# clevercool/ANT-Quantization

Measured on AMD Instinct MI355X. Metric: Gelements/s quant-dequant + achieved HBM GB/s %peak, 4-bit ANT, 1/8 MI355X, higher is better.
Workload: dtype f32; 1 GPU; headline: 32 x [4096,4096] bf16 weight tensors per GPU, ANT 4-bit signed flint grid, calibrated per-row alpha, steady-state _forward; one step = ONE batched launch (antq_fakequant_batch) over all 32 tensors; io_dtype=bf16

## Files before the change

### ant_quantization_amd/_lib.py

```python
import ctypes
import os
import threading

import numpy as np
import torch

_HERE = os.path.dirname(os.path.abspath(__file__))
LIB_PATH = os.environ.get("ANTQ_LIB") or os.path.join(_HERE, "libantq.so")

ABI_VERSION = 7
F32, BF16, F16, F64 = 0, 1, 2, 3
FLAG_OVP = 1
FLAG_DYNAMIC = 2
FLAG_UNORDERED = 4
IDX_NONE = -1
IDX_VICTIM = -2
MAX_GRID = 1024
PLAN_MAX_BYTES = 128 + 4 * MAX_GRID + 16 * 3072 + 20 * 1024 + 16 * 64

_DTYPES = {torch.float32: F32, torch.bfloat16: BF16, torch.float16: F16, torch.float64: F64}

_lib = None
_lock = threading.RLock()

# ... 799 lines not shown
            else:
                batched.append(j)
        self.n_batched = len(batched)
        self.host = self.dev = None
        if batched:
            arr = (_Job * len(batched))()
            for k, (x, out, alpha, plan, gmax, rows, row_len, per_row) in enumerate(batched):
                arr[k] = _Job(x.data_ptr(), out.data_ptr(), alpha.data_ptr() if alpha is not None else 0, rows, row_len,
                              1 if per_row else 0, gmax,
                              plan.host_addr, plan.dev(self.device).data_ptr())
            cap = lib().antq_batch_capacity(arr, len(batched), self.dtype)
            host = np.zeros(cap, dtype=np.uint8)
            n = lib().antq_batch_build(arr, len(batched), self.dtype,
                                       (FLAG_OVP if ovp else 0) | (FLAG_DYNAMIC if dynamic else 0),
                                       host.ctypes.data_as(ctypes.c_void_p), ctypes.c_size_t(cap))
            if n <= 0:
                _check(n, "antq_batch_build")
            self.host = host[:n].copy()
            self.dev = torch.from_numpy(self.host).to(self.device)

    def run(self):
        e = _ext_mod if _ext_mod is not False else ext()
        if self.host is not None and e is not None:
            e.batch_run(self.host.ctypes.data, self.dev)
        elif self.host is not None:
            with _on_device(self.device):
                rc = lib().antq_fakequant_batch(ctypes.c_void_p(self.host.ctypes.data), ctypes.c_void_p(self.dev.data_ptr()),
                                                ctypes.c_void_p(_stream_int(self.device)))
            if rc:
                _check(rc, "antq_fakequant_batch")
        for x, out, alpha, plan, gmax, rows, row_len, per_row in self.singles:
            fakequant(x, alpha, plan, gmax, rows, row_len, per_row, ovp=self.ovp, out=out)

    def kernels(self):
        out = []
        if self.host is not None:
            h = self.host[:80].view(np.uint32)
            fam, pad = [int(v) for v in h[8:17]], int(h[17])
            t = {F32: "float", BF16: "bf16", F16: "f16"}[self.dtype]
            o = "true" if self.ovp else "false"
            dyn = "true" if int(h[3]) & FLAG_DYNAMIC else "false"
            if pad & 1:
                out.append(("antq::k_fq_batch_all<%s,%s>" % (t, o), fam[0]))
            elif fam[0]:
                w = 1 if ((pad >> 8) & 7) == 1 else 4
                out.append(("antq::k_fq_batch<%s,%s,%d>" % (t, o, w), fam[0] * (4 // w)))
            if fam[5]:
                out.append(("antq::k_fq_hbatch<%s,%s>" % (t, o), fam[5] * 4))
            for f, v in ((6, 1), (7, 4), (8, 16)):
                if fam[f] and not (pad & 1):
                    out.append(("antq::k_fq_hbatch_dyn<%s,%s,%d>" % (t, o, v), fam[f]))
            if not (pad & 1):
                if fam[1]:
                    out.append(("antq::k_fq_batch_d<%s,%s,true,%s>" % (t, o, dyn), fam[1]))
                if fam[2]:
                    out.append(("antq::k_fq_batch_d<%s,%s,false,%s>" % (t, o, dyn), fam[2]))
                if fam[3]:
                    out.append(("antq::k_fq_batch_dyn<%s,%s>" % (t, o), fam[3]))
                if fam[4]:
                    out.append(("antq::k_fq_batch_dyn16<%s,%s>" % (t, o), fam[4]))
        out += [("antq_fakequant (own launch)", 0)] * len(self.singles)
        return out
```

### ant_quantization_amd/csrc/antq_batch.hip

```cpp
#include "antq_host.h"
#include "antq_k_batch.h"

using namespace antq;

extern "C" size_t antq_batch_capacity(const antq_job *jobs, int n, int dtype)
{
    const int epl = epl_of(dtype);
    if (!jobs || n < 1 || !epl) return 0;
    size_t blocks = 0;
    for (int i = 0; i < n; i++) blocks += std::max(4 * job_blocks(jobs[i], epl, nullptr) + 1, jobs[i].rows);
    return sizeof(BatchHeader) + sizeof(BatchDesc) * (size_t)n + 4 * blocks;
}

extern "C" int antq_batch_build(const antq_job *jobs, int n, int dtype, unsigned flags, void *blob, size_t cap)
{
    const int epl = epl_of(dtype);
    if (!jobs || !blob || n < 1 || n > 65535) return ANTQ_ERR_ARG;
    if (!epl) return ANTQ_ERR_UNSUPPORTED;
    const bool dyn = (flags & ANTQ_FLAG_DYNAMIC) != 0;
    char *p = static_cast<char *>(blob);
    BatchHeader h;
    memset(&h, 0, sizeof(h));
    h.magic = kBatchMagic; h.n = (uint32_t)n; h.dtype = (uint32_t)dtype; h.flags = flags;
    h.map_offset = (uint32_t)(sizeof(BatchHeader) + sizeof(BatchDesc) * (size_t)n);
// ... 19 lines not shown
        if (!plan_args_from_host(J.plan_host, d.pa)) return ANTQ_ERR_PLAN;
        const PlanHeader *ph = static_cast<const PlanHeader *>(J.plan_host);
        const bool xdom = g_knob_x && d.pa.kind == kPlanLut && ph->xdom;
        d.vout = ph->vout;
        {
            const XArgs xe = xargs_from_plan(J.plan_host, d.pa);
            d.vmin = xe.vmin; d.vmax = xe.vmax;
        }
        d.ratio = 1.0f;
        int f;
        d.u = (uint32_t)kBatchU;
        if (!dyn) {
            if (d.kind == 0 && d.pa.adom && (dtype == ANTQ_F32 || g_knob_lane_rows == 2) && g_knob_lane_rows != 0) {
                d.kind = 1; d.total_tasks = 0; d.tpr = 1; d.vshift = -1;
                if ((d.vpr & (d.vpr - 1u)) == 0u) { d.vshift = 0; while ((1u << d.vshift) < d.vpr) d.vshift++; }
                blocks = (size_t)((d.n_vec + 256u * kBatchU - 1u) / (256u * kBatchU));
            }
            HArgs hx;
            const uint32_t hu = (d.kind == 0 && g_knob_h != 0 && hargs_from_plan(J.plan_host, dtype, J.gmax, hx))
                                    ? (g_knob_h == 2 ? row_task_u(d.vpr) : hrow_static_u(d.vpr, xdom)) : 0u;
            if (hu != 0u) {
                d.kind = 13;
                d.u = hu;
                if (g_knob_u >= 2 && g_knob_u <= 4) d.u = (uint32_t)g_knob_u;
                d.tpr = (d.vpr + 64u * d.u - 1u) / (64u * d.u);
                const size_t total = (J.alpha_per_row ? J.rows : (size_t)1) * (size_t)d.tpr;
                if (total > 0xfffffff0ull) return ANTQ_ERR_UNSUPPORTED;
                d.total_tasks = (uint32_t)total;
                blocks = (total + 3) / 4;
                d.rot = (d.vpr % (64u * d.u) != 0u && (d.tpr % 2u) == 0u) ? 1u : 0u;
                d.tlist = plan_tlist_dev(J.plan_host, J.plan_dev);
                d.h_n = hx.n_thr | (hx.n_neg << 16);
                d.hshift = hx.hshift;
            }
            if (d.kind == 0 && xdom) {
                d.kind = 2;
                d.u = row_task_u_small(d.vpr);
                if (g_knob_u >= 1 && g_knob_u <= 4) d.u = (uint32_t)g_knob_u;
                d.tpr = (d.vpr + 64u * d.u - 1u) / (64u * d.u);
                const size_t total = (J.alpha_per_row ? J.rows : (size_t)1) * (size_t)d.tpr;
                if (total > 0xfffffff0ull) return ANTQ_ERR_UNSUPPORTED;
                d.total_tasks = (uint32_t)total;
                blocks = (total + 3) / 4;
                d.rot = (d.vpr % (64u * d.u) != 0u && (d.tpr % 2u) == 0u) ? 1u : 0u;
            }
            f = d.kind == 13 ? 5 : d.kind == 2 ? 0 : (d.kind == 3 ? -1 : (d.pa.adom ? 1 : 2));
        } else {
            if (!J.alpha_per_row || d.kind == 3 || J.rows > 0x3ffffff0ull) return ANTQ_ERR_UNSUPPORTED;
            HArgs hprobe;
            const bool h_dyn = d.kind == 0 && g_knob_h != 0 && d.vpr <= 8192u && hargs_from_plan(J.plan_host, dtype, J.gmax, hprobe);
            if (!h_dyn && d.kind == 0 && d.pa.adom && dtype != ANTQ_F32 && d.vpr == 128u && g_knob_u != 1) {
                d.kind = 1; d.total_tasks = 0; d.tpr = 1; d.vshift = 7;
                blocks = (size_t)((d.n_vec + 256u * kBatchU - 1u) / (256u * kBatchU));
            }
            const HArgs &hx = hprobe;
            if (h_dyn) {
                const HDynShape sh = hrow_dyn_shape(d.vpr);
                d.kind = sh.wpr == 1 ? 14 : (sh.wpr == 4 ? 15 : 16);
                d.u = (uint32_t)sh.vpt;
                d.tpr = (uint32_t)sh.wpr;
                d.total_tasks = (uint32_t)(J.rows * (size_t)sh.wpr);
                blocks = sh.wpr == 1 ? (J.rows + 3) / 4 : J.rows;
                d.tlist = plan_tlist_dev(J.plan_host, J.plan_dev);
                d.h_n = hx.n_thr | (hx.n_neg << 16);
                d.hshift = hx.hshift;
                f = sh.wpr == 1 ? 6 : (sh.wpr == 4 ? 7 : 8);
// ... 30 lines not shown
        d.inv_gmax = 1.0 / (double)J.gmax;
        descs[i] = d;
        fam[(size_t)i] = (uint8_t)(f < 0 ? 255 : f);
        nblk[(size_t)i] = blocks;
        if (f == 1 || f == 2 || f < 0) lds = std::max(lds, lds_table(d.pa, false));
    }
    for (int i = 0; i < n; i++)
        if (fam[(size_t)i] == 255) fam[(size_t)i] = any_da ? 1 : 2;
    {
        size_t all_blocks = 0;
        for (int i = 0; i < n; i++) all_blocks += nblk[(size_t)i];
        const bool small = g_knob_u == 2 || (g_knob_u != 4 && (all_blocks < 4u * 2048u || dtype == ANTQ_F32));
        for (int i = 0; i < n && small; i++) {
            BatchDesc &d = descs[i];
            if (d.kind == 1 && d.pa.adom && !(dyn && d.vpr > 64u)) {
                d.u = 2u;
                nblk[(size_t)i] = (size_t)((d.n_vec + 511u) / 512u);
            }
        }
    }
    if (!dyn) {
        double h_bytes = 0.0;
        for (int i = 0; i < n; i++)
            if (fam[(size_t)i] == 5) h_bytes += 2.0 * (double)jobs[i].rows * (double)jobs[i].row_len * (dtype == ANTQ_F32 ? 4.0 : 2.0);
        const bool h_apart = h_bytes >= 128.0 * 1048576.0;
        if (!h_apart) {
            for (int i = 0; i < n; i++) {
                BatchDesc &d = descs[i];
                if (d.kind != 13) continue;
                bool other = false;
                for (int k = 0; k < n && !other; k++) other = fam[(size_t)k] != 5;
                if (!other) break;
                const PlanHeader *ph = static_cast<const PlanHeader *>(jobs[i].plan_host);
                if (g_knob_x && d.pa.kind == kPlanLut && ph->xdom) {
                    d.kind = 2;
                    d.u = row_task_u_small(d.vpr);
                    d.tpr = (d.vpr + 64u * d.u - 1u) / (64u * d.u);
                    d.total_tasks = (uint32_t)((jobs[i].alpha_per_row ? jobs[i].rows : (size_t)1) * (size_t)d.tpr);
                    d.rot = (d.vpr % (64u * d.u) != 0u && (d.tpr % 2u) == 0u) ? 1u : 0u;
                    fam[(size_t)i] = 0;
                } else {
                    const size_t tpr = (d.vpr + 64 * kBatchU - 1) / (64 * kBatchU);
                    d.kind = 0; d.u = (uint32_t)kBatchU; d.tpr = (uint32_t)tpr; d.rot = 0;
                    d.total_tasks = (uint32_t)((jobs[i].alpha_per_row ? jobs[i].rows : (size_t)1) * tpr);
                    lds = std::max(lds, lds_table(d.pa, false));
                    fam[(size_t)i] = (uint8_t)(d.pa.adom ? 1 : 2);
                }
                nblk[(size_t)i] = ((size_t)d.total_tasks + 3) / 4;
            }
        }
        bool seen[kBatchFamilies] = {false, false, false, false, false, false, false, false, false};
        int nf_rest = 0;
        for (int i = 0; i < n; i++)
            if (fam[(size_t)i] != 5 && !seen[fam[(size_t)i]]) { seen[fam[(size_t)i]] = true; nf_rest++; }
        if (nf_rest > 1) {
            h.pad = 1u;
            for (int i = 0; i < n; i++)
                if (fam[(size_t)i] != 5) fam[(size_t)i] = 0;
        }
    }
    {
        double long_b = 0.0, short_b = 0.0;
        for (int i = 0; i < n; i++)
            if (descs[i].kind == 2) (descs[i].vpr >= 256u ? long_b : short_b) += (double)descs[i].total_tasks * descs[i].u;
        h.pad |= ((long_b >= short_b && !big_footprint) ? 1u : 4u) << 8;
    }
    {
        uint32_t umax = 0;
        for (int i = 0; i < n; i++)
            if (descs[i].kind == 14) umax = std::max(umax, descs[i].u);
        h.pad2[0] = hrow_dyn_lds_pad(HDynShape{1, (int)umax});
    }
    size_t total_blocks = 0;
    for (int i = 0; i < n; i++) {
        descs[i].first_block = (uint32_t)fam_blocks[fam[(size_t)i]];
        fam_blocks[fam[(size_t)i]] += nblk[(size_t)i];
        total_blocks += nblk[(size_t)i];
    }
    if (total_blocks > 0x1fffffffull) return ANTQ_ERR_UNSUPPORTED;
    if (cap < h.map_offset + 4 * total_blocks) return ANTQ_ERR_PLAN;
    size_t off[kBatchFamilies], acc = 0;
    for (int f = 0; f < kBatchFamilies; f++) { off[f] = acc; acc += fam_blocks[f]; h.fam_blocks[f] = (uint32_t)fam_blocks[f]; }
    for (int i = 0; i < n; i++) {
        uint32_t *m = map + off[fam[(size_t)i]] + descs[i].first_block;
        for (size_t b = 0; b < nblk[(size_t)i]; b++) m[b] = (uint32_t)i;
    }
    h.total_blocks = (uint32_t)total_blocks;
    h.lds_bytes = (uint32_t)lds;
    h.bytes = (uint32_t)(h.map_offset + 4 * total_blocks);
    memcpy(p, &h, sizeof(h));
    return (int)h.bytes;
}

template <typename T>
static void launch_hbatch(uint32_t map_entries, const BatchDesc *descs, const uint32_t *map, bool ovp, hipStream_t st)
{
    const dim3 g(map_entries * 4u), b(64u);
    const unsigned pad = g_knob_hlds >= 0 ? (unsigned)g_knob_hlds : (map_entries >= 8192u ? kHRowLdsPad : 0u);
    if (ovp) hipLaunchKernelGGL((k_fq_hbatch<T, true>), g, b, pad, st, descs, map, (uint32_t)g_knob_rot);
    else hipLaunchKernelGGL((k_fq_hbatch<T, false>), g, b, pad, st, descs, map, (uint32_t)g_knob_rot);
}
template <>
void launch_hbatch<float>(uint32_t, const BatchDesc *, const uint32_t *, bool, hipStream_t) {}

template <typename T>
static void launch_hbatch_dyn(const BatchHeader *h, const BatchDesc *descs, const uint32_t *const *fmap, bool ovp, hipStream_t st)
{
    if (h->fam_blocks[6]) {
        const dim3 g(h->fam_blocks[6] * 4u), b(64u);
        const unsigned pad = g_knob_hlds >= 0 ? (unsigned)g_knob_hlds : h->pad2[0];
        if (ovp) hipLaunchKernelGGL((k_fq_hbatch_dyn<T, true, 1>), g, b, pad, st, descs, fmap[6]);
        else hipLaunchKernelGGL((k_fq_hbatch_dyn<T, false, 1>), g, b, pad, st, descs, fmap[6]);
    }
    if (h->fam_blocks[7]) {
        const dim3 g(h->fam_blocks[7]), b(256u);
        if (ovp) hipLaunchKernelGGL((k_fq_hbatch_dyn<T, true, 4>), g, b, 0, st, descs, fmap[7]);
        else hipLaunchKernelGGL((k_fq_hbatch_dyn<T, false, 4>), g, b, 0, st, descs, fmap[7]);
    }
    if (h->fam_blocks[8]) {
        const dim3 g(h->fam_blocks[8]), b(1024u);
        if (ovp) hipLaunchKernelGGL((k_fq_hbatch_dyn<T, true, 16>), g, b, 0, st, descs, fmap[8]);
        else hipLaunchKernelGGL((k_fq_hbatch_dyn<T, false, 16>), g, b, 0, st, descs, fmap[8]);
    }
}
template <>
void launch_hbatch_dyn<float>(const BatchHeader *, const BatchDesc *, const uint32_t *const *, bool, hipStream_t) {}

extern "C" int antq_fakequant_batch(const void *batch_host, const void *batch_dev, void *stream)
{
    if (!batch_host || !batch_dev) return ANTQ_ERR_ARG;
    const BatchHeader *h = static_cast<const BatchHeader *>(batch_host);
    if (h->magic != kBatchMagic) return ANTQ_ERR_PLAN;
    if (h->total_blocks == 0) return ANTQ_OK;
    const char *pd = static_cast<const char *>(batch_dev);
    const BatchDesc *descs = reinterpret_cast<const BatchDesc *>(pd + sizeof(BatchHeader));
    const uint32_t *map = reinterpret_cast<const uint32_t *>(pd + h->map_offset);
    hipStream_t st = static_cast<hipStream_t>(stream);
    const dim3 block(256);
    const bool ovp = (h->flags & ANTQ_FLAG_OVP) != 0;
    const bool dyn = (h->flags & ANTQ_FLAG_DYNAMIC) != 0;
    const uint32_t *fmap[kBatchFamilies];
    {
        const uint32_t *m = map;
        for (int f = 0; f < kBatchFamilies; f++) { fmap[f] = m; m += h->fam_blocks[f]; }
    }
#define ANTQ_LAUNCH_D(TT, OO, AA)                                                                                   \
    do {                                                                                                            \
        const int f_ = (AA) ? 1 : 2;                                                                                \
         \
        const unsigned cap_ = (sizeof(TT) == 4 && !dyn && h->fam_blocks[f_] >= 32768u && h->lds_bytes < 24576u) ? 24576u - h->lds_bytes : 0u;  \
        const unsigned lds_ = h->lds_bytes + (g_knob_dlds >= 0 ? (unsigned)g_knob_dlds : cap_);                    \
        if (dyn) hipLaunchKernelGGL((k_fq_batch_d<TT, OO, AA, true>), dim3(h->fam_blocks[f_]), block, lds_, st, descs, fmap[f_]);  \
        else hipLaunchKernelGGL((k_fq_batch_d<TT, OO, AA, false>), dim3(h->fam_blocks[f_]), block, lds_, st, descs, fmap[f_]);     \
    } while (0)
#define ANTQ_LAUNCH_B(TT)                                                                                         \
    do {                                                                                                          \
        if (h->pad & 1u) {                                             \
            if (ovp) hipLaunchKernelGGL((k_fq_batch_all<TT, true>), dim3(h->fam_blocks[0]), block, h->lds_bytes, st, descs, fmap[0]);  \
            else hipLaunchKernelGGL((k_fq_batch_all<TT, false>), dim3(h->fam_blocks[0]), block, h->lds_bytes, st, descs, fmap[0]);     \
            if (h->fam_blocks[5]) launch_hbatch<TT>(h->fam_blocks[5], descs, fmap[5], ovp, st);    \
            break;                                                                                                \
        }                                                                                                         \
        if (h->fam_blocks[0]) {                                                                                   \
            const int hw_ = (int)((h->pad >> 8) & 7u);                                                           \
            const int w_ = (g_knob_waves == 4 || g_knob_waves == 2 || g_knob_waves == 1) ? g_knob_waves : (hw_ == 1 ? 1 : 4);   \
            const dim3 g_(h->fam_blocks[0] * (4u / w_)), b_(64u * w_);                                           \
            const uint32_t rot_ = (uint32_t)g_knob_rot;                                                          \
            if (w_ == 1) { if (ovp) hipLaunchKernelGGL((k_fq_batch<TT, true, 1>), g_, b_, 0, st, descs, fmap[0], rot_);        \
                           else hipLaunchKernelGGL((k_fq_batch<TT, false, 1>), g_, b_, 0, st, descs, fmap[0], rot_); }         \
            else if (w_ == 2) { if (ovp) hipLaunchKernelGGL((k_fq_batch<TT, true, 2>), g_, b_, 0, st, descs, fmap[0], rot_);   \
                           else hipLaunchKernelGGL((k_fq_batch<TT, false, 2>), g_, b_, 0, st, descs, fmap[0], rot_); }         \
            else { if (ovp) hipLaunchKernelGGL((k_fq_batch<TT, true, 4>), g_, b_, 0, st, descs, fmap[0], rot_);                \
                   else hipLaunchKernelGGL((k_fq_batch<TT, false, 4>), g_, b_, 0, st, descs, fmap[0], rot_); }                 \
        }                                                                                                         \
        if (h->fam_blocks[5]) launch_hbatch<TT>(h->fam_blocks[5], descs, fmap[5], ovp, st);                       \
        if (h->fam_blocks[6] || h->fam_blocks[7] || h->fam_blocks[8]) launch_hbatch_dyn<TT>(h, descs, fmap, ovp, st);      \
        if (h->fam_blocks[1]) { if (ovp) ANTQ_LAUNCH_D(TT, true, true); else ANTQ_LAUNCH_D(TT, false, true); }    \
        if (h->fam_blocks[2]) { if (ovp) ANTQ_LAUNCH_D(TT, true, false); else ANTQ_LAUNCH_D(TT, false, false); }  \
        if (h->fam_blocks[3]) {                                                                                   \
            if (ovp) hipLaunchKernelGGL((k_fq_batch_dyn<TT, true>), dim3(h->fam_blocks[3]), block, 0, st, descs, fmap[3]);   \
            else hipLaunchKernelGGL((k_fq_batch_dyn<TT, false>), dim3(h->fam_blocks[3]), block, 0, st, descs, fmap[3]);      \
        }                                                                                                         \
        if (h->fam_blocks[4]) {                                                                                   \
            if (ovp) hipLaunchKernelGGL((k_fq_batch_dyn16<TT, true>), dim3(h->fam_blocks[4]), dim3(1024), 0, st, descs, fmap[4]);   \
            else hipLaunchKernelGGL((k_fq_batch_dyn16<TT, false>), dim3(h->fam_blocks[4]), dim3(1024), 0, st, descs, fmap[4]);      \
        }                                                                                                         \
    } while (0)
    switch (h->dtype) {
    case ANTQ_F32: ANTQ_LAUNCH_B(float); break;
    case ANTQ_BF16: ANTQ_LAUNCH_B(bf16_tag); break;
    case ANTQ_F16: ANTQ_LAUNCH_B(f16_tag); break;
    default: return ANTQ_ERR_UNSUPPORTED;
    }
#undef ANTQ_LAUNCH_B
#undef ANTQ_LAUNCH_D
    return hipGetLastError() == hipSuccess ? ANTQ_OK : ANTQ_ERR_LAUNCH;
}

namespace antq {
int prefetch_unit_batch()
{
    hipFuncAttributes at;
    return hipFuncGetAttributes(&at, reinterpret_cast<const void *>(&k_fq_hbatch<bf16_tag, false>)) == hipSuccess ? ANTQ_OK : ANTQ_ERR_LAUNCH;
}
}
```

### ant_quantization_amd/csrc/antq_k_batch.h

```cpp
#ifndef ANTQ_K_BATCH_H
#define ANTQ_K_BATCH_H

#include "antq_k_fakequant.h"
#include "antq_k_hrow.h"

namespace antq {

constexpr uint32_t kBatchMagic = 0x33544E41u;
constexpr int kBatchU = 4;

struct BatchDesc {
    const uint4 *x;
    uint4 *out;
    const float *alpha;
    const uint4 *plan_tab;
    uint64_t n_vec;
    uint32_t total_tasks;
    uint32_t vpr;
    uint32_t tpr;
    int32_t vshift;
    uint32_t first_block;
    uint32_t kind;
    int32_t per_row;
    float gmax;
    PlanArgs pa;
    float vout;
    float ratio;
    uint32_t u;
    uint32_t rot;
    float vmin, vmax;
    uint32_t pad_;
    double inv_gmax;
    const uint4 *tlist;
    uint32_t h_n;
    uint32_t hshift;
};
static_assert(sizeof(BatchDesc) == 192, "BatchDesc must be 192 bytes");

constexpr int kBatchFamilies = 9;

struct BatchHeader {
    uint32_t magic, n, dtype, flags, lds_bytes, map_offset, bytes, total_blocks;
    uint32_t fam_blocks[kBatchFamilies];
    uint32_t pad;
    uint32_t pad2[2];
};
static_assert(sizeof(BatchHeader) == 80, "BatchHeader must be 80 bytes");

__device__ __forceinline__ XArgs xargs_of(const BatchDesc &D)
{
    const PlanArgs &pa = D.pa;
    XArgs xa;
    xa.m = pa.m; xa.shift = pa.shift; xa.kmin = pa.kmin; xa.kmax = pa.kmax; xa.keymask = pa.keymask;
    xa.nbneg = pa.nbneg; xa.n_entries = pa.n_entries; xa.xlim = pa.xlim; xa.vout = D.vout;
    xa.linear = pa.linear; xa.lin_scale = pa.lin_scale; xa.lin_bias = pa.lin_bias;
    xa.flim = pa.fastlim * 0.99999f; xa.vmin = D.vmin; xa.vmax = D.vmax; xa.inv_gmax = D.inv_gmax;
    return xa;
}

#ifndef ANTQ_OVP_WAVES
#define ANTQ_OVP_WAVES 8
#endif
#ifndef ANTQ_PLAIN_WAVES
#define ANTQ_PLAIN_WAVES 6
#endif
template <typename T, bool OVP, int WAVES = 4>
__global__ void __launch_bounds__(64 * WAVES, OVP ? ANTQ_OVP_WAVES : ANTQ_PLAIN_WAVES)
k_fq_batch(const BatchDesc *__restrict__ descs, const uint32_t *__restrict__ block_map, uint32_t rotate)
{
    constexpr uint32_t SPLIT = 4u / WAVES;
    uint32_t blk = blockIdx.x;
    if (WAVES < 4) {
        const uint32_t g8 = blk >> 3;
        if ((g8 << 3) + 8u <= gridDim.x && (rotate == 1u || (rotate == 0u && descs[block_map[(g8 << 3) / SPLIT]].rot)))
            blk = (g8 << 3) + ((blk + g8) & 7u);
    }
    const uint32_t b4 = blk / SPLIT, sub = blk % SPLIT;
    const uint32_t j = block_map[b4];
    const BatchDesc &D = descs[j];
    const uint32_t lb = b4 - D.first_block;
    const uint32_t lane = threadIdx.x & 63u;
    const uint32_t wv = threadIdx.x >> 6;
    const uint4 *plan_tab = D.plan_tab;
    const XArgs xa = xargs_of(D);

    __shared__ __attribute__((aligned(16))) uint4 wtab_all[WAVES][256];
    const uint32_t task = __builtin_amdgcn_readfirstlane(lb * 4u + sub * WAVES + wv);
    if (task >= D.total_tasks) return;
#define ANTQ_XROW(UU)                                                                                                   \
    xrow_task<T, OVP, false, UU, false, 1>(D.x, D.out, nullptr, task, D.vpr, D.tpr, D.alpha, D.per_row, D.gmax, 1.0f, nullptr, \
                                           xa, plan_tab + (D.pa.m_pad >> 2), reinterpret_cast<const float *>(plan_tab),        \
                                           wtab_all[wv], lane, wv)
    if (D.u == 4u) ANTQ_XROW(4); else if (D.u == 3u) ANTQ_XROW(3); else if (D.u == 1u) ANTQ_XROW(1); else ANTQ_XROW(2);
#undef ANTQ_XROW
}

template <typename T, bool OVP>
__global__ void __launch_bounds__(64)
k_fq_hbatch(const BatchDesc *__restrict__ descs, const uint32_t *__restrict__ block_map, uint32_t rotate)
{
    __shared__ __attribute__((aligned(16))) uint2 tab[kHSlots * 2];
    uint32_t blk = blockIdx.x;
    const uint32_t g8 = blk >> 3;
    if ((g8 << 3) + 8u <= gridDim.x && (rotate == 1u || (rotate == 0u && descs[block_map[(g8 << 3) >> 2]].rot)))
        blk = (g8 << 3) + ((blk + g8) & 7u);
    const uint32_t b4 = blk >> 2, sub = blk & 3u;
    const BatchDesc &D = descs[block_map[b4]];
    const uint32_t task = (b4 - D.first_block) * 4u + sub;
    if (task >= D.total_tasks) return;
    HArgs ha;
    ha.n_thr = D.h_n & 0xffffu; ha.n_neg = D.h_n >> 16; ha.hshift = D.hshift; ha.m = D.pa.m;
    ha.flim = D.pa.fastlim * 0.99999f; ha.lim = fminf(ha.flim, D.pa.xlim);
    ha.vmin = D.vmin; ha.vmax = D.vmax; ha.vout = D.vout; ha.inv_gmax = D.inv_gmax;
    const float *grid = reinterpret_cast<const float *>(D.plan_tab);
#define ANTQ_HROW(UU) hrow_wave_task<T, OVP, UU>(D.x, D.out, task, D.vpr, D.tpr, D.alpha, D.per_row, D.gmax, ha, D.tlist, grid, tab, threadIdx.x)
    if (D.u == 4u) ANTQ_HROW(4); else if (D.u == 3u) ANTQ_HROW(3); else ANTQ_HROW(2);
#undef ANTQ_HROW
}

template <typename T, bool OVP, int WPR>
__global__ void __launch_bounds__(64 * WPR)
k_fq_hbatch_dyn(const BatchDesc *__restrict__ descs, const uint32_t *__restrict__ block_map)
{
    __shared__ __attribute__((aligned(16))) uint2 tab[WPR][kHSlots * 2];
    const uint32_t wv = threadIdx.x >> 6, lane = threadIdx.x & 63u;
    const uint32_t ent = WPR == 1 ? (blockIdx.x >> 2) : blockIdx.x;
    const BatchDesc &D = descs[block_map[ent]];
    const uint32_t rowi = WPR == 1 ? (ent - D.first_block) * 4u + (blockIdx.x & 3u) : ent - D.first_block;
    if (rowi * (uint32_t)WPR >= D.total_tasks) return;
    const uint32_t task = __builtin_amdgcn_readfirstlane(rowi * WPR + wv);
    HArgs ha;
    ha.n_thr = D.h_n & 0xffffu; ha.n_neg = D.h_n >> 16; ha.hshift = D.hshift; ha.m = D.pa.m;
    ha.flim = D.pa.fastlim * 0.99999f; ha.lim = fminf(ha.flim, D.pa.xlim);
    ha.vmin = D.vmin; ha.vmax = D.vmax; ha.vout = D.vout; ha.inv_gmax = D.inv_gmax;
    const float *grid = reinterpret_cast<const float *>(D.plan_tab);
    float *alpha_out = const_cast<float *>(D.alpha);
    hrow_wave_task_dyn<T, OVP, WPR>(D.x, D.out, task, D.vpr, D.u, D.ratio, alpha_out, D.gmax, ha, D.tlist, grid, tab[wv], lane, wv);
}

template <typename T, bool OVP, bool AD, bool DYN>
__global__ void __launch_bounds__(256)
k_fq_batch_d(const BatchDesc *__restrict__ descs, const uint32_t *__restrict__ block_map)
{
    constexpr int U = kBatchU;
    extern __shared__ __attribute__((aligned(16))) uint4 smem[];
    const uint32_t j = block_map[blockIdx.x];
    const BatchDesc &D = descs[j];
    const PlanArgs pa = D.pa;
    const uint32_t lb = blockIdx.x - D.first_block;
// ... 207 lines not shown
```

### ant_quantization_amd/csrc/antq_k_hrow.h

```cpp
#ifndef ANTQ_K_HROW_H
#define ANTQ_K_HROW_H

#include "antq_k_fakequant.h"

namespace antq {

constexpr uint32_t kHNoThr = 0xffffffffu;
constexpr uint32_t kHSentinel = 0xffffu;

struct HArgs {
    uint32_t n_thr;
    uint32_t n_neg;
    uint32_t hshift;
    uint32_t m;
    float lim;
    float flim;
    float vmin, vmax;
    float vout;
    double inv_gmax;
};

template <typename T> struct H16;
template <> struct H16<bf16_tag> {
    static constexpr uint32_t MANT = 7;
// ... 78 lines not shown
    }
    __builtin_amdgcn_fence(__ATOMIC_RELEASE, "wavefront");
    __builtin_amdgcn_wave_barrier();
    __builtin_amdgcn_s_waitcnt(0xc07f);
    return R;
}

__device__ __forceinline__ uint32_t hrow_pair(uint32_t w, uint32_t tbase, uint32_t vkmin, uint32_t vklim, uint32_t kpos,
                                               uint32_t vkwid)
{
    uint32_t th, tl, wl, o;
    uint2 eh, el;
    asm("v_bfe_u32 %0, %1, %2, %3" : "=v"(th) : "v"(w), "s"(kpos), "v"(vkwid));
    asm("v_med3_i32 %0, %1, %2, %3" : "=v"(th) : "v"(th), "v"(vkmin), "v"(vklim));
    wl = w << 16;
    th = __builtin_amdgcn_alignbit(th, w, 31);
    asm("v_bfe_u32 %0, %1, %2, %3" : "=v"(tl) : "v"(wl), "s"(kpos), "v"(vkwid));
    asm("v_med3_i32 %0, %1, %2, %3" : "=v"(tl) : "v"(tl), "v"(vkmin), "v"(vklim));
    tl = __builtin_amdgcn_alignbit(tl, wl, 31);
    typedef unsigned int u32x2_t __attribute__((ext_vector_type(2)));
    const u32x2_t rh = *(const __attribute__((address_space(3))) u32x2_t *)(uintptr_t)((th << 3) + tbase);
    const u32x2_t rl = *(const __attribute__((address_space(3))) u32x2_t *)(uintptr_t)((tl << 3) + tbase);
    eh = make_uint2(rh.x, rh.y);
    el = make_uint2(rl.x, rl.y);
    asm("v_cmp_ge_u32 vcc, %1, %2\n\t"
        "v_cndmask_b32_sdwa %0, %3, %3, vcc dst_sel:DWORD dst_unused:UNUSED_PAD src0_sel:WORD_0 src1_sel:WORD_1"
        : "=&v"(o) : "v"(wl), "v"(el.x), "v"(el.y) : "vcc");
    asm("v_cmp_ge_u32 vcc, %1, %2\n\t"
        "v_cndmask_b32_sdwa %0, %3, %3, vcc dst_sel:WORD_1 dst_unused:UNUSED_PRESERVE src0_sel:WORD_0 src1_sel:WORD_1"
        : "+v"(o) : "v"(w), "v"(eh.x), "v"(eh.y) : "vcc");
    return o;
}

__device__ __forceinline__ uint32_t vec_word(const uint4 &v, int i) { return i == 0 ? v.x : (i == 1 ? v.y : (i == 2 ? v.z : v.w)); }
__device__ __forceinline__ void vec_set(uint4 &v, int i, uint32_t w)
{
    if (i == 0) v.x = w; else if (i == 1) v.y = w; else if (i == 2) v.z = w; else v.w = w;
}

template <typename T, bool OVP>
__device__ __forceinline__ uint4 hrow_exact(const uint4 &v, float s, const float *__restrict__ grid, uint32_t m)
{
    uint4 o = v;
#pragma unroll 1
    for (int i = 0; i < 4; i++) {
        const uint32_t w = vec_word(v, i);
        const float x0 = H16<T>::val(w & 0xffffu), x1 = H16<T>::val(w >> 16);
        const float d0 = x0 / s, d1 = x1 / s;
        float q0 = 0.0f, q1 = 0.0f, m0 = 102400.0f, m1 = 102400.0f;
#pragma unroll 1
        for (uint32_t k = 0; k < m; k++) {
            const float g = ld_global(grid + k);
            const float s0 = fabsf(d0 - g), s1 = fabsf(d1 - g);
            if (s0 <= m0) { m0 = s0; q0 = g; }
            if (s1 <= m1) { m1 = s1; q1 = g; }
        }
        if (OVP) {
            const bool me = fabsf(q0) > 32.0f, mo = fabsf(q1) > 32.0f;
            q0 = q0 * ((mo && !me) ? 0.0f : 1.0f);
            q1 = q1 * (me ? 0.0f : 1.0f);
        }
        const float t0 = (q0 - d0) + d0, t1 = (q1 - d1) + d1;
        vec_set(o, i, H16<T>::out(t0 * s) | (H16<T>::out(t1 * s) << 16));
    }
    return o;
}

__device__ __forceinline__ uint32_t hrow_victims(uint32_t o, uint32_t othr)
{
    const uint32_t mg = o & 0x7fff7fffu;
    const bool me = (mg & 0xffffu) >= othr, mo = (mg >> 16) >= othr;
    return o & (((mo && !me) ? 0u : 0xffffu) | (me ? 0u : 0xffff0000u));
}

struct HFar { float rs, flim, vmin, vmax; };

template <typename T, bool OVP>
__device__ __forceinline__ uint4 hrow_vec_far(const uint4 &v, uint32_t tbase, uint32_t vkmin, uint32_t vklim, uint32_t kpos,
                                              uint32_t vkwid, uint32_t othr, float s, const HFar &far,
                                              const float *__restrict__ grid, uint32_t m)
{
    uint4 o = v;
    bool decided = true;
#pragma unroll 1
    for (int i = 0; i < 4; i++) {
        const uint32_t w = vec_word(v, i);
        uint32_t ow = hrow_pair(w, tbase, vkmin, vklim, kpos, vkwid);
#pragma unroll
        for (int hf = 0; hf < 2; hf++) {
            if (((ow >> (16 * hf)) & 0xffffu) == kHSentinel) {
                const float xe = H16<T>::val((w >> (16 * hf)) & 0xffffu);
                decided = decided && (fabsf(xe * far.rs) < far.flim);
                const float d = xe / s;
                const float q = (d > 0.0f ? far.vmax : far.vmin) + 0.0f;
                const float t = (q - d) + d;
                const uint32_t pat = H16<T>::out(t * s);
                ow = hf ? ((ow & 0xffffu) | (pat << 16)) : ((ow & 0xffff0000u) | pat);
            }
        }
        if (OVP) ow = hrow_victims(ow, othr);
        vec_set(o, i, ow);
    }
    if (!decided) return hrow_exact<T, OVP>(v, s, grid, m);
    return o;
}

template <typename T, bool OVP, int VPT>
__device__ __forceinline__ void hrow_task(const uint4 (&v)[VPT], uint4 *__restrict__ out, uint32_t v0, uint32_t vpr,
                                          const HRow &R, uint32_t tab_addr, uint32_t hshift, uint32_t othr, float s,
                                          const HFar &far, const float *__restrict__ grid, uint32_t m, uint32_t nv = VPT)
{
    const uint32_t kpos = 16u + hshift;
    uint32_t vkmin = R.kmin, vklim = R.klim, vkwid = 15u - hshift;
    asm volatile("" : "+v"(vkmin), "+v"(vklim), "+v"(vkwid));
    const uint32_t tbase = tab_addr - (R.kmin << 4);
    if (R.fast) {
        u16x2_t acc = as_u16x2(0u);
#pragma unroll
        for (int u = 0; u < VPT; u++) {
            if ((uint32_t)u < nv && v0 + 64u * u < vpr) {
                const uint32_t w[4] = {v[u].x, v[u].y, v[u].z, v[u].w};
                uint32_t o[4];
#pragma unroll
                for (int i = 0; i < 4; i++) {
                    o[i] = hrow_pair(w[i], tbase, vkmin, vklim, kpos, vkwid);
                    acc = __builtin_elementwise_max(acc, as_u16x2(o[i]));
                    if (OVP) o[i] = hrow_victims(o[i], othr);
                }
                st_stream(out + 64u * u, make_uint4(o[0], o[1], o[2], o[3]));
            }
            __builtin_amdgcn_sched_barrier(0);
        }
        const uint32_t na = ~as_u32(acc);
        if (__builtin_expect((na & 0xffffu) != 0u && (na >> 16) != 0u, 1)) return;
    }
    const uint32_t slot0 = R.klim << hshift;
#pragma unroll 1
    for (uint32_t u = 0; u < nv; u++) {
        uint4 cur = v[0];
#pragma unroll
        for (int k = 1; k < VPT; k++)
            if (u == (uint32_t)k) cur = v[k];
        if (v0 + 64u * u < vpr) {
            const uint32_t top = IO<T>::amax_acc(0u, cur);
            if (!R.fast) st_stream(out + 64u * u, hrow_exact<T, OVP>(cur, s, grid, m));
            else if (max(top & 0xffffu, top >> 16) >= slot0)
                st_stream(out + 64u * u, hrow_vec_far<T, OVP>(cur, tbase, vkmin, vklim, kpos, vkwid, othr, s, far, grid, m));
        }
    }
}

constexpr unsigned kHRowLdsPad = 6656u - kHSlots * 16u;

template <typename T, bool OVP, int VPT>
__device__ __forceinline__ void hrow_wave_finish(const uint4 (&v)[VPT], uint4 *__restrict__ out, uint32_t v0, uint32_t vpr,
                                                 float a, float gmax, const HArgs &ha, const uint4 &thr,
                                                 const float *__restrict__ grid, uint2 *tab, uint32_t lane, uint32_t nv = VPT)
{
    const Scale sc = row_scale(a, gmax, ha.inv_gmax);
    HRow R = hrow_build<T>(ha, thr, sc, tab, lane);
    const uint32_t othr = OVP ? H16<T>::out(ha.vout * sc.s) & 0x7fffu : 0u;
    if (OVP && othr >= H16<T>::INF && ha.vout < __builtin_inff()) R.fast = false;
    const uint32_t tab_addr = (uint32_t)(uintptr_t)(__attribute__((address_space(3))) void *)tab;
    const HFar far = {sc.rs, ha.flim, ha.vmin, ha.vmax};
    hrow_task<T, OVP, VPT>(v, out, v0, vpr, R, tab_addr, ha.hshift, othr, sc.s, far, grid, ha.m, nv);
}

template <typename T, bool OVP, int VPT>
__device__ __forceinline__ void hrow_wave_task(const uint4 *__restrict__ x, uint4 *__restrict__ out, uint32_t task, uint32_t vpr,
                                               uint32_t tpr, const float *__restrict__ alpha, int per_row, float gmax,
                                               const HArgs &ha, const uint4 *__restrict__ tlist, const float *__restrict__ grid,
                                               uint2 *tab, uint32_t lane)
{
    constexpr uint32_t nv = VPT;
    uint32_t row = task, g = 0;
    if (tpr != 1) { row = task / tpr; g = task - row * tpr; }
    uint4 thr = ld_global(tlist + min(lane, ha.n_thr - 1u));
    const float a = ld_global(alpha + (per_row ? row : 0));
    const uint32_t v0 = g * (64u * nv) + lane;
    const uint4 *p = x + (size_t)row * vpr;
    uint4 v[VPT];
#pragma unroll
    for (int u = 0; u < VPT; u++) v[u] = ld_stream(p + min(v0 + 64u * u, vpr - 1u));
    __builtin_amdgcn_sched_barrier(0);
    asm volatile("" : "+v"(thr.x), "+v"(thr.y), "+v"(thr.z), "+v"(thr.w));
    hrow_wave_finish<T, OVP, VPT>(v, out + (size_t)row * vpr + v0, v0, vpr, a, gmax, ha, thr, grid, tab, lane, nv);
}

constexpr int kHDynV = 8;
template <typename T, bool OVP, int WPR>
__device__ __forceinline__ void hrow_wave_task_dyn(const uint4 *__restrict__ x, uint4 *__restrict__ out, uint32_t task, uint32_t vpr,
                                                   uint32_t nv, float ratio, float *__restrict__ alpha_out, float gmax,
                                                   const HArgs &ha, const uint4 *__restrict__ tlist, const float *__restrict__ grid,
                                                   uint2 *tab, uint32_t lane, uint32_t wv)
{
    const uint32_t row = WPR == 1 ? task : task / WPR, g = WPR == 1 ? 0u : task - row * WPR;
    uint4 thr = ld_global(tlist + min(lane, ha.n_thr - 1u));
    const uint32_t v0 = g * (64u * nv) + lane;
    const uint4 *p = x + (size_t)row * vpr;
    uint4 v[kHDynV];
#pragma unroll
    for (int u = 0; u < kHDynV; u++) {
        v[u] = make_uint4(0u, 0u, 0u, 0u);
        if ((uint32_t)u < nv) v[u] = ld_stream(p + min(v0 + 64u * u, vpr - 1u));
    }
    __builtin_amdgcn_sched_barrier(0);
    asm volatile("" : "+v"(thr.x), "+v"(thr.y), "+v"(thr.z), "+v"(thr.w));
    uint32_t m = 0;
#pragma unroll
    for (int u = 0; u < kHDynV; u++)
        if ((uint32_t)u < nv && v0 + 64u * u < vpr) m = IO<T>::amax_acc(m, v[u]);
    m = wave_max_u32(IO<T>::amax_bits(m));
    if (WPR > 1) {
        __shared__ uint32_t wmax[WPR];
        if (lane == 0) wmax[wv] = m;
        __syncthreads();
        m = wmax[0];
#pragma unroll
        for (int w = 1; w < WPR; w++) m = max(m, wmax[w]);
// ... 42 lines not shown
    return lds > kHSlots * 16u ? lds - kHSlots * 16u : 0u;
}

template <typename T, bool OVP, int VPT, int WAVES = 1>
__global__ void __launch_bounds__(64 * WAVES)
k_fq_hrow(const uint4 *__restrict__ x, uint4 *__restrict__ out, uint32_t total_tasks, uint32_t vpr, uint32_t tpr,
          const float *__restrict__ alpha, int per_row, float gmax, HArgs ha, const uint4 *__restrict__ tlist,
          const float *__restrict__ grid)
{
    __shared__ __attribute__((aligned(16))) uint2 tab[WAVES][kHSlots * 2];
    const uint32_t wv = threadIdx.x >> 6;
    const uint32_t task = __builtin_amdgcn_readfirstlane(blockIdx.x * WAVES + wv);
    if (task >= total_tasks) return;
    hrow_wave_task<T, OVP, VPT>(x, out, task, vpr, tpr, alpha, per_row, gmax, ha, tlist, grid, tab[wv], threadIdx.x & 63u);
}

static inline bool hargs_from_plan(const void *plan_host, int dtype, float gmax, HArgs &ha)
{
    const PlanHeader *ph = static_cast<const PlanHeader *>(plan_host);
    const int t = dtype == ANTQ_BF16 ? 0 : dtype == ANTQ_F16 ? 1 : -1;
    if (t < 0 || ph->kind != kPlanLut || !(ph->hdom & (1u << t))) return false;
    ha.n_thr = ph->h_nthr; ha.n_neg = ph->h_nneg;
    ha.hshift = (ph->hshift >> (8 * t)) & 0xffu;
    ha.m = ph->m;
    ha.flim = ph->fastlim * 0.99999f;
    ha.lim = ha.flim < ph->xlim ? ha.flim : ph->xlim;
    const float *g = plan_grid(plan_host);
    ha.vmin = ha.vmax = g[0];
    for (uint32_t i = 1; i < ph->m; i++) { ha.vmin = g[i] < ha.vmin ? g[i] : ha.vmin; ha.vmax = g[i] > ha.vmax ? g[i] : ha.vmax; }
    ha.vout = ph->vout;
    ha.inv_gmax = 1.0 / (double)gmax;
    return true;
}
static inline const uint4 *plan_tlist_dev(const void *plan_host, const void *plan_dev)
{
    return reinterpret_cast<const uint4 *>(static_cast<const char *>(plan_dev) + static_cast<const PlanHeader *>(plan_host)->tlist_off);
}


}

#endif
```

Baseline: 1642 Gelem/s.

## Add direct-indexed LDS lookup table for per-row hbatch quantization

```diff
diff --git a/ant_quantization_amd/_lib.py b/ant_quantization_amd/_lib.py
--- a/ant_quantization_amd/_lib.py
+++ b/ant_quantization_amd/_lib.py
@@ -855,6 +855,13 @@
         for x, out, alpha, plan, gmax, rows, row_len, per_row in self.singles:
             fakequant(x, alpha, plan, gmax, rows, row_len, per_row, ovp=self.ovp, out=out)
 
+    def table_forms(self):
+        if self.host is None:
+            return []
+        n = int(self.host[:80].view(np.uint32)[1])
+        d = [self.host[80 + 192 * i:80 + 192 * (i + 1)].view(np.uint32) for i in range(n)]
+        return [(int(w[15]), int(w[41])) for w in d]
+
     def kernels(self):
         out = []
         if self.host is not None:
diff --git a/ant_quantization_amd/csrc/antq_batch.hip b/ant_quantization_amd/csrc/antq_batch.hip
--- a/ant_quantization_amd/csrc/antq_batch.hip
+++ b/ant_quantization_amd/csrc/antq_batch.hip
@@ -75,6 +75,7 @@
                 d.tlist = plan_tlist_dev(J.plan_host, J.plan_dev);
                 d.h_n = hx.n_thr | (hx.n_neg << 16);
                 d.hshift = hx.hshift;
+                d.h_cap = g_knob_h == 3 ? 0u : hrow_direct_cap(J.plan_host, dtype, hx);
             }
             if (d.kind == 0 && xdom) {
                 d.kind = 2;
@@ -171,6 +172,7 @@
                 for (int k = 0; k < n && !other; k++) other = fam[(size_t)k] != 5;
                 if (!other) break;
                 const PlanHeader *ph = static_cast<const PlanHeader *>(jobs[i].plan_host);
+                d.h_cap = 0u;
                 if (g_knob_x && d.pa.kind == kPlanLut && ph->xdom) {
                     d.kind = 2;
                     d.u = row_task_u_small(d.vpr);
@@ -209,6 +211,11 @@
         for (int i = 0; i < n; i++)
             if (descs[i].kind == 14) umax = std::max(umax, descs[i].u);
         h.pad2[0] = hrow_dyn_lds_pad(HDynShape{1, (int)umax});
+        uint32_t hneed = 0;
+        for (int i = 0; i < n; i++) {
+            if (descs[i].kind == 13) hneed = std::max(hneed, descs[i].h_cap ? (kHDirHead + descs[i].h_cap) * 4u : kHSlots * 16u);
+        }
+        h.pad2[1] = hneed;
     }
     size_t total_blocks = 0;
     for (int i = 0; i < n; i++) {
@@ -232,15 +239,16 @@
 }
 
 template <typename T>
-static void launch_hbatch(uint32_t map_entries, const BatchDesc *descs, const uint32_t *map, bool ovp, hipStream_t st)
+static void launch_hbatch(uint32_t map_entries, uint32_t need, const BatchDesc *descs, const uint32_t *map, bool ovp, hipStream_t st)
 {
     const dim3 g(map_entries * 4u), b(64u);
     const unsigned pad = g_knob_hlds >= 0 ? (unsigned)g_knob_hlds : (map_entries >= 8192u ? kHRowLdsPad : 0u);
-    if (ovp) hipLaunchKernelGGL((k_fq_hbatch<T, true>), g, b, pad, st, descs, map, (uint32_t)g_knob_rot);
-    else hipLaunchKernelGGL((k_fq_hbatch<T, false>), g, b, pad, st, descs, map, (uint32_t)g_knob_rot);
+    const unsigned lds = std::max(need, kHSlots * 16u + pad);
+    if (ovp) hipLaunchKernelGGL((k_fq_hbatch<T, true>), g, b, lds, st, descs, map, (uint32_t)g_knob_rot);
+    else hipLaunchKernelGGL((k_fq_hbatch<T, false>), g, b, lds, st, descs, map, (uint32_t)g_knob_rot);
 }
 template <>
-void launch_hbatch<float>(uint32_t, const BatchDesc *, const uint32_t *, bool, hipStream_t) {}
+void launch_hbatch<float>(uint32_t, uint32_t, const BatchDesc *, const uint32_t *, bool, hipStream_t) {}
 
 template <typename T>
 static void launch_hbatch_dyn(const BatchHeader *h, const BatchDesc *descs, const uint32_t *const *fmap, bool ovp, hipStream_t st)
@@ -297,7 +305,7 @@
         if (h->pad & 1u) {                                             \
             if (ovp) hipLaunchKernelGGL((k_fq_batch_all<TT, true>), dim3(h->fam_blocks[0]), block, h->lds_bytes, st, descs, fmap[0]);  \
             else hipLaunchKernelGGL((k_fq_batch_all<TT, false>), dim3(h->fam_blocks[0]), block, h->lds_bytes, st, descs, fmap[0]);     \
-            if (h->fam_blocks[5]) launch_hbatch<TT>(h->fam_blocks[5], descs, fmap[5], ovp, st);    \
+            if (h->fam_blocks[5]) launch_hbatch<TT>(h->fam_blocks[5], h->pad2[1], descs, fmap[5], ovp, st);    \
             break;                                                                                                \
         }                                                                                                         \
         if (h->fam_blocks[0]) {                                                                                   \
@@ -312,7 +320,7 @@
             else { if (ovp) hipLaunchKernelGGL((k_fq_batch<TT, true, 4>), g_, b_, 0, st, descs, fmap[0], rot_);                \
                    else hipLaunchKernelGGL((k_fq_batch<TT, false, 4>), g_, b_, 0, st, descs, fmap[0], rot_); }                 \
         }                                                                                                         \
-        if (h->fam_blocks[5]) launch_hbatch<TT>(h->fam_blocks[5], descs, fmap[5], ovp, st);                       \
+        if (h->fam_blocks[5]) launch_hbatch<TT>(h->fam_blocks[5], h->pad2[1], descs, fmap[5], ovp, st);                       \
         if (h->fam_blocks[6] || h->fam_blocks[7] || h->fam_blocks[8]) launch_hbatch_dyn<TT>(h, descs, fmap, ovp, st);      \
         if (h->fam_blocks[1]) { if (ovp) ANTQ_LAUNCH_D(TT, true, true); else ANTQ_LAUNCH_D(TT, false, true); }    \
         if (h->fam_blocks[2]) { if (ovp) ANTQ_LAUNCH_D(TT, true, false); else ANTQ_LAUNCH_D(TT, false, false); }  \
diff --git a/ant_quantization_amd/csrc/antq_k_batch.h b/ant_quantization_amd/csrc/antq_k_batch.h
--- a/ant_quantization_amd/csrc/antq_k_batch.h
+++ b/ant_quantization_amd/csrc/antq_k_batch.h
@@ -29,13 +29,14 @@
     uint32_t u;
     uint32_t rot;
     float vmin, vmax;
-    uint32_t pad_;
+    uint32_t h_cap;
     double inv_gmax;
     const uint4 *tlist;
     uint32_t h_n;
     uint32_t hshift;
 };
 static_assert(sizeof(BatchDesc) == 192, "BatchDesc must be 192 bytes");
+static_assert(offsetof(BatchDesc, kind) == 60 && offsetof(BatchDesc, h_cap) == 164, "BatchDesc layout (Batch.table_forms reads these)");
 
 constexpr int kBatchFamilies = 9;
 
@@ -99,7 +100,7 @@
 __global__ void __launch_bounds__(64)
 k_fq_hbatch(const BatchDesc *__restrict__ descs, const uint32_t *__restrict__ block_map, uint32_t rotate)
 {
-    __shared__ __attribute__((aligned(16))) uint2 tab[kHSlots * 2];
+    extern __shared__ __attribute__((aligned(16))) uint2 tab[];
     uint32_t blk = blockIdx.x;
     const uint32_t g8 = blk >> 3;
     if ((g8 << 3) + 8u <= gridDim.x && (rotate == 1u || (rotate == 0u && descs[block_map[(g8 << 3) >> 2]].rot)))
@@ -113,8 +114,11 @@
     ha.flim = D.pa.fastlim * 0.99999f; ha.lim = fminf(ha.flim, D.pa.xlim);
     ha.vmin = D.vmin; ha.vmax = D.vmax; ha.vout = D.vout; ha.inv_gmax = D.inv_gmax;
     const float *grid = reinterpret_cast<const float *>(D.plan_tab);
-#define ANTQ_HROW(UU) hrow_wave_task<T, OVP, UU>(D.x, D.out, task, D.vpr, D.tpr, D.alpha, D.per_row, D.gmax, ha, D.tlist, grid, tab, threadIdx.x)
-    if (D.u == 4u) ANTQ_HROW(4); else if (D.u == 3u) ANTQ_HROW(3); else ANTQ_HROW(2);
+#define ANTQ_HROW(UU, DD)                                                                                                \
+    hrow_wave_task<T, OVP, UU, DD>(D.x, D.out, task, D.vpr, D.tpr, D.alpha, D.per_row, D.gmax, ha, D.tlist, grid, tab,  \
+                                   threadIdx.x, D.h_cap)
+    if (D.h_cap != 0u) { if (D.u == 4u) ANTQ_HROW(4, true); else if (D.u == 3u) ANTQ_HROW(3, true); else ANTQ_HROW(2, true); }
+    else if (D.u == 4u) ANTQ_HROW(4, false); else if (D.u == 3u) ANTQ_HROW(3, false); else ANTQ_HROW(2, false);
 #undef ANTQ_HROW
 }
 
diff --git a/ant_quantization_amd/csrc/antq_k_hrow.h b/ant_quantization_amd/csrc/antq_k_hrow.h
--- a/ant_quantization_amd/csrc/antq_k_hrow.h
+++ b/ant_quantization_amd/csrc/antq_k_hrow.h
@@ -134,6 +134,115 @@
     return o;
 }
 
+constexpr uint32_t kHDirHead = 256;
+constexpr uint32_t kHDirMaxEntries = 1408;
+
+__device__ __forceinline__ uint32_t wave_scan_add_u32(uint32_t x)
+{
+#define ANTQ_DPP_ADD(CTRL, ROWS) x += (uint32_t)__builtin_amdgcn_update_dpp(0, (int)x, CTRL, ROWS, 0xf, false)
+    ANTQ_DPP_ADD(0x111, 0xf);
+    ANTQ_DPP_ADD(0x112, 0xf);
+    ANTQ_DPP_ADD(0x114, 0xf);
+    ANTQ_DPP_ADD(0x118, 0xf);
+    ANTQ_DPP_ADD(0x142, 0xa);
+    ANTQ_DPP_ADD(0x143, 0xc);
+#undef ANTQ_DPP_ADD
+    return x;
+}
+
+__device__ __forceinline__ void hrow_lds_sync()
+{
+    __builtin_amdgcn_fence(__ATOMIC_RELEASE, "wavefront");
+    __builtin_amdgcn_wave_barrier();
+    __builtin_amdgcn_s_waitcnt(0xc07f);
+}
+
+template <typename T>
+__device__ __forceinline__ HRow hrow_build_direct(const HArgs &ha, const uint4 &thr, const Scale &sc, uint32_t *lds, uint32_t cap,
+                                                  uint32_t lane)
+{
+    HRow R;
+    const float s = sc.s;
+    bool ok = sc.ok && (s > 0.0f);
+    const bool mine = lane < ha.n_thr;
+    const bool neg = lane < ha.n_neg;
+    const float limx = ha.lim * s * 0.999f;
+    const uint32_t lim16 = (uint32_t)__builtin_amdgcn_readfirstlane((int)(ok ? H16<T>::down(fminf(limx, 3.0e38f)) : 0u));
+    bool tok;
+    const float Tt = mine ? u2f(thr.x) : 1.0f;
+    const float U = x_threshold(Tt, ok ? s : 1.0f, sc.rs, tok);
+    const uint32_t t16 = neg ? H16<T>::down(-U) + 1u : H16<T>::up(U);
+    const uint32_t o_lo = H16<T>::out((u2f(thr.y) + 0.0f) * s), o_hi = H16<T>::out((u2f(thr.z) + 0.0f) * s);
+    const uint32_t first = neg ? o_hi : o_lo, second = neg ? o_lo : o_hi;
+    const uint32_t t_prev = (uint32_t)__shfl((int)t16, (int)((lane + 63u) & 63u), 64);
+    const uint32_t t_next = (uint32_t)__shfl((int)t16, (int)((lane + 1u) & 63u), 64);
+    const bool last_of_side = neg ? (lane == 0u) : (lane + 1u == ha.n_thr);
+    const bool first_of_side = neg ? (lane + 1u == ha.n_neg) : (lane == ha.n_neg);
+    const uint32_t nxt = last_of_side ? lim16 : (neg ? t_prev : t_next);
+    const uint32_t tpos = ha.n_neg < ha.n_thr ? (uint32_t)__builtin_amdgcn_readlane((int)t16, (int)ha.n_neg) : 0xffffffffu;
+    const uint32_t tneg = ha.n_neg > 0u ? (uint32_t)__builtin_amdgcn_readlane((int)t16, (int)(ha.n_neg - 1u)) : 0xffffffffu;
+    const uint32_t tmin = min(tpos, tneg);
+    const uint32_t p0 = tmin - 1u;
+    const uint32_t n = lim16 - p0 + 1u;
+    const bool lane_ok = !mine || (t16 < nxt);
+    ok = ok && (tmin >= 1u) && (lim16 >= tmin) && (n <= cap) && (__ballot(lane_ok) == ~0ull);
+    R.kmin = p0; R.klim = lim16; R.fast = ok;
+    if (!ok) return R;
+    const uint32_t pshift = n <= 1024u ? 4u : (n <= 2048u ? 5u : 6u);
+    uint32_t *cnt = lds, *opos = lds + 64, *oneg = lds + 129, *ent = lds + kHDirHead;
+    cnt[lane] = 0u;
+    hrow_lds_sync();
+    const uint32_t idx = t16 - p0;
+    if (mine) {
+        __hip_atomic_fetch_add(cnt + (idx >> pshift), neg ? 0x10000u : 1u, __ATOMIC_RELAXED, __HIP_MEMORY_SCOPE_WAVEFRONT);
+        uint32_t *o = neg ? oneg : opos;
+        o[(neg ? ha.n_neg - 1u - lane : lane - ha.n_neg) + 1u] = second;
+        if (first_of_side) o[0] = first;
+    }
+    if (ha.n_neg == 0u || ha.n_neg == ha.n_thr) {
+        const bool ng = ha.n_neg == 0u;
+        const uint32_t o = (uint32_t)__builtin_amdgcn_readlane((int)first, ng ? 0 : (int)(ha.n_thr - 1u));
+        if (lane == 0u) (ng ? oneg : opos)[0] = o;
+    }
+    hrow_lds_sync();
+    const uint32_t c = cnt[lane];
+    const uint32_t before = wave_scan_add_u32(c) - c;
+    const uint32_t e = opos[before & 0xffffu] | (oneg[before >> 16] << 16);
+    if ((lane << pshift) < n) {
+        uint4 *q = reinterpret_cast<uint4 *>(ent + (lane << pshift));
+#pragma clang loop unroll(disable)
+        for (uint32_t j = 0; j < (1u << (pshift - 2u)); j++) q[j] = make_uint4(e, e, e, e);
+    }
+    hrow_lds_sync();
+    if (mine) {
+        const uint32_t len = min(nxt - p0, ((idx >> pshift) + 1u) << pshift) - idx;
+        uint16_t *hp = reinterpret_cast<uint16_t *>(ent + idx) + (neg ? 1 : 0);
+        for (uint32_t j0 = 0; j0 < (1u << pshift); j0 += 16u) {
+#pragma unroll
+            for (uint32_t j = 0; j < 16u; j++)
+                if (j0 + j < len) hp[2u * (j0 + j)] = (uint16_t)second;
+        }
+    }
+    hrow_lds_sync();
+    if (lane == 0u) ent[n - 1u] = 0xffffffffu;
+    hrow_lds_sync();
+    return R;
+}
+
+__device__ __forceinline__ uint32_t hrow_pair_direct(uint32_t w, uint32_t ebase, uint32_t p0x2, uint32_t lastx2)
+{
+    u16x2_t c = __builtin_elementwise_sub_sat(as_u16x2(w & 0x7fff7fffu), as_u16x2(p0x2));
+    c = __builtin_elementwise_min(c, as_u16x2(lastx2));
+    uint32_t p, al, ah;
+    asm("v_and_or_b32 %0, %1, %2, %3" : "=v"(p) : "v"(w >> 14), "s"(0x00020002u), "v"(as_u32(c << 2)));
+    asm("v_add_u32_sdwa %0, %1, %2 dst_sel:DWORD dst_unused:UNUSED_PAD src0_sel:WORD_0 src1_sel:DWORD" : "=v"(al) : "v"(p), "v"(ebase));
+    asm("v_add_u32_sdwa %0, %1, %2 dst_sel:DWORD dst_unused:UNUSED_PAD src0_sel:WORD_1 src1_sel:DWORD" : "=v"(ah) : "v"(p), "v"(ebase));
+    typedef const __attribute__((address_space(3))) unsigned short *lds_u16_t;
+    const uint32_t lo = *(lds_u16_t)(uintptr_t)al;
+    const uint32_t hi = *(lds_u16_t)(uintptr_t)ah;
+    return lo | (hi << 16);
+}
+
 __device__ __forceinline__ uint32_t vec_word(const uint4 &v, int i) { return i == 0 ? v.x : (i == 1 ? v.y : (i == 2 ? v.z : v.w)); }
 __device__ __forceinline__ void vec_set(uint4 &v, int i, uint32_t w)
 {
@@ -177,7 +286,7 @@
 
 struct HFar { float rs, flim, vmin, vmax; };
 
-template <typename T, bool OVP>
+template <typename T, bool OVP, bool DIRECT = false>
 __device__ __forceinline__ uint4 hrow_vec_far(const uint4 &v, uint32_t tbase, uint32_t vkmin, uint32_t vklim, uint32_t kpos,
                                               uint32_t vkwid, uint32_t othr, float s, const HFar &far,
                                               const float *__restrict__ grid, uint32_t m)
@@ -187,7 +296,7 @@
 #pragma unroll 1
     for (int i = 0; i < 4; i++) {
         const uint32_t w = vec_word(v, i);
-        uint32_t ow = hrow_pair(w, tbase, vkmin, vklim, kpos, vkwid);
+        uint32_t ow = DIRECT ? hrow_pair_direct(w, tbase, vkmin, vklim) : hrow_pair(w, tbase, vkmin, vklim, kpos, vkwid);
 #pragma unroll
         for (int hf = 0; hf < 2; hf++) {
             if (((ow >> (16 * hf)) & 0xffffu) == kHSentinel) {
@@ -207,15 +316,15 @@
     return o;
 }
 
-template <typename T, bool OVP, int VPT>
+template <typename T, bool OVP, int VPT, bool DIRECT = false>
 __device__ __forceinline__ void hrow_task(const uint4 (&v)[VPT], uint4 *__restrict__ out, uint32_t v0, uint32_t vpr,
                                           const HRow &R, uint32_t tab_addr, uint32_t hshift, uint32_t othr, float s,
                                           const HFar &far, const float *__restrict__ grid, uint32_t m, uint32_t nv = VPT)
 {
     const uint32_t kpos = 16u + hshift;
-    uint32_t vkmin = R.kmin, vklim = R.klim, vkwid = 15u - hshift;
+    uint32_t vkmin = DIRECT ? R.kmin * 0x10001u : R.kmin, vklim = DIRECT ? (R.klim - R.kmin) * 0x10001u : R.klim, vkwid = 15u - hshift;
     asm volatile("" : "+v"(vkmin), "+v"(vklim), "+v"(vkwid));
-    const uint32_t tbase = tab_addr - (R.kmin << 4);
+    const uint32_t tbase = DIRECT ? tab_addr + 4u * kHDirHead : tab_addr - (R.kmin << 4);
     if (R.fast) {
         u16x2_t acc = as_u16x2(0u);
 #pragma unroll
@@ -225,7 +334,7 @@
                 uint32_t o[4];
 #pragma unroll
                 for (int i = 0; i < 4; i++) {
-                    o[i] = hrow_pair(w[i], tbase, vkmin, vklim, kpos, vkwid);
+                    o[i] = DIRECT ? hrow_pair_direct(w[i], tbase, vkmin, vklim) : hrow_pair(w[i], tbase, vkmin, vklim, kpos, vkwid);
                     acc = __builtin_elementwise_max(acc, as_u16x2(o[i]));
                     if (OVP) o[i] = hrow_victims(o[i], othr);
                 }
@@ -236,7 +345,7 @@
         const uint32_t na = ~as_u32(acc);
         if (__builtin_expect((na & 0xffffu) != 0u && (na >> 16) != 0u, 1)) return;
     }
-    const uint32_t slot0 = R.klim << hshift;
+    const uint32_t slot0 = DIRECT ? R.klim : R.klim << hshift;
 #pragma unroll 1
     for (uint32_t u = 0; u < nv; u++) {
         uint4 cur = v[0];
@@ -247,32 +356,34 @@
             const uint32_t top = IO<T>::amax_acc(0u, cur);
             if (!R.fast) st_stream(out + 64u * u, hrow_exact<T, OVP>(cur, s, grid, m));
             else if (max(top & 0xffffu, top >> 16) >= slot0)
-                st_stream(out + 64u * u, hrow_vec_far<T, OVP>(cur, tbase, vkmin, vklim, kpos, vkwid, othr, s, far, grid, m));
+                st_stream(out + 64u * u, hrow_vec_far<T, OVP, DIRECT>(cur, tbase, vkmin, vklim, kpos, vkwid, othr, s, far, grid, m));
         }
     }
 }
 
 constexpr unsigned kHRowLdsPad = 6656u - kHSlots * 16u;
 
-template <typename T, bool OVP, int VPT>
+template <typename T, bool OVP, int VPT, bool DIRECT = false>
 __device__ __forceinline__ void hrow_wave_finish(const uint4 (&v)[VPT], uint4 *__restrict__ out, uint32_t v0, uint32_t vpr,
                                                  float a, float gmax, const HArgs &ha, const uint4 &thr,
-                                                 const float *__restrict__ grid, uint2 *tab, uint32_t lane, uint32_t nv = VPT)
+                                                 const float *__restrict__ grid, uint2 *tab, uint32_t lane, uint32_t nv = VPT,
+                                                 uint32_t cap = 0u)
 {
     const Scale sc = row_scale(a, gmax, ha.inv_gmax);
-    HRow R = hrow_build<T>(ha, thr, sc, tab, lane);
+    HRow R = DIRECT ? hrow_build_direct<T>(ha, thr, sc, reinterpret_cast<uint32_t *>(tab), cap, lane)
+                    : hrow_build<T>(ha, thr, sc, tab, lane);
     const uint32_t othr = OVP ? H16<T>::out(ha.vout * sc.s) & 0x7fffu : 0u;
     if (OVP && othr >= H16<T>::INF && ha.vout < __builtin_inff()) R.fast = false;
     const uint32_t tab_addr = (uint32_t)(uintptr_t)(__attribute__((address_space(3))) void *)tab;
     const HFar far = {sc.rs, ha.flim, ha.vmin, ha.vmax};
-    hrow_task<T, OVP, VPT>(v, out, v0, vpr, R, tab_addr, ha.hshift, othr, sc.s, far, grid, ha.m, nv);
-}
-
-template <typename T, bool OVP, int VPT>
+    hrow_task<T, OVP, VPT, DIRECT>(v, out, v0, vpr, R, tab_addr, ha.hshift, othr, sc.s, far, grid, ha.m, nv);
+}
+
+template <typename T, bool OVP, int VPT, bool DIRECT = false>
 __device__ __forceinline__ void hrow_wave_task(const uint4 *__restrict__ x, uint4 *__restrict__ out, uint32_t task, uint32_t vpr,
                                                uint32_t tpr, const float *__restrict__ alpha, int per_row, float gmax,
                                                const HArgs &ha, const uint4 *__restrict__ tlist, const float *__restrict__ grid,
-                                               uint2 *tab, uint32_t lane)
+                                               uint2 *tab, uint32_t lane, uint32_t cap = 0u)
 {
     constexpr uint32_t nv = VPT;
     uint32_t row = task, g = 0;
@@ -286,7 +397,7 @@
     for (int u = 0; u < VPT; u++) v[u] = ld_stream(p + min(v0 + 64u * u, vpr - 1u));
     __builtin_amdgcn_sched_barrier(0);
     asm volatile("" : "+v"(thr.x), "+v"(thr.y), "+v"(thr.z), "+v"(thr.w));
-    hrow_wave_finish<T, OVP, VPT>(v, out + (size_t)row * vpr + v0, v0, vpr, a, gmax, ha, thr, grid, tab, lane, nv);
+    hrow_wave_finish<T, OVP, VPT, DIRECT>(v, out + (size_t)row * vpr + v0, v0, vpr, a, gmax, ha, thr, grid, tab, lane, nv, cap);
 }
 
 constexpr int kHDynV = 8;
@@ -395,6 +506,17 @@
     ha.inv_gmax = 1.0 / (double)gmax;
     return true;
 }
+static inline uint32_t hrow_direct_cap(const void *plan_host, int dtype, const HArgs &ha)
+{
+    const HThr *tl = plan_tlist(plan_host);
+    double tmin = INFINITY;
+    for (uint32_t i = 0; i < ha.n_thr; i++) tmin = std::min(tmin, fabs((double)tl[i].T));
+    const double lim = (double)ha.lim * 0.999;
+    if (!(tmin > 0.0) || !(lim > tmin)) return 0u;
+    const double e = (dtype == ANTQ_BF16 ? 128.0 : 1024.0) * (log2(lim / tmin) + 1.0) + 4.0;
+    if (!(e <= (double)kHDirMaxEntries)) return 0u;
+    return ((uint32_t)ceil(e) + 63u) & ~63u;
+}
 static inline const uint4 *plan_tlist_dev(const void *plan_host, const void *plan_dev)
 {
     return reinterpret_cast<const uint4 *>(static_cast<const char *>(plan_dev) + static_cast<const PlanHeader *>(plan_host)->tlist_off);
```

Result: no change. 1646 Gelem/s, median of 6 (+0.2%).
